# flo-stilz/Audio-Key-Estimation

Measured on AMD Instinct MI355X. Metric: clips/s (15 s @ 22.05 kHz), HIP CQT + PitchClassNet forward, higher is better.
Workload: dtype f32 accumulation everywhere; pitch / semitone / layer-0 convolutions: f16 activations x f16 weights (per-channel power-of-two scaled) on MFMA, one product; last layer's pitch-class convolutions and heads: 3-term split-bf16 on MFMA (hi*hi + lo*hi + hi*lo); CQT filter bank: 3-term split-bf16 on MFMA

## Files before the change

audio-key-estimation_amd/csrc/pcnet.hip:

```cpp
#include <algorithm>
#include <cmath>
#include <cstdlib>
#include <cstring>
#include <map>
#include <string>
#include <vector>

#include "common.h"
#include "pcnet_kernels.h"
#include "pcnet_bwd_kernels.h"

using namespace ake_k;

namespace {

constexpr double kBnEps = 1e-5;
constexpr size_t kLdsBudget = 64 * 1024;
constexpr size_t kBfFragsPerConv = 14 * 2 * 64 + 64;

struct TensorSpec {
    std::string name;
    int64_t shape[4];
    int ndim;
};
// ... 620 lines not shown
        if (j == 0) { a.ph = melh; a.uh = psix_h; a.c0 = 1; a.c1 = c1; a.h1 = 36; }
        else a.xh = planes[j - 1];
        if (!fold) a.oh = planes[j];
        else {
            a.sfrag = n->bf_frags_dev + semi.bf_off; a.sbias = n->blob_dev + semi.b_off;
            a.n_oct = g.n_oct; a.n_units = batch * (36 / a.R);
            a.dst = cat + static_cast<long long>(fold_coff) * 12 * T;
            a.dst_clip_stride = static_cast<long long>(cat_ctot) * 12 * T;
        }
    }
    static ake::DeviceOnce attr_set;
    const int rc = ake::raise_lds_limit(attr_set, 160 * 1024, p2p_stack_kernel);
    if (rc) return rc;
    return ake::launch(name, p2p_stack_kernel, dim3(batch), dim3(1024), g.lds, s, sa);
}

struct P2pX3Plan {
    bool ok = false;
    int R = 0, plane_pos = 0, n_row_tiles = 0, n_tiles = 0, grid = 0;
    size_t lds = 0;
};
P2pX3Plan p2p_f16x3_plan(int c0, int c1, int cout, int batch, int H, int T, bool dst16) {
    P2pX3Plan g;
    if (T < 2 || (T & 1) || c0 < 1 || c0 + c1 > 8 || cout > 8 || batch < 1) return g;
    const int n_cus = device_cus();
    if (n_cus < 8) return g;
    const int Tp = p2p_pitch(T / 2);
    auto plane_of = [&](int R) { return ((R + 6) * Tp + 63) / 64 * 64; };
    auto lds_of = [&](int R) { return (static_cast<size_t>(4) * plane_of(R) + 8 * kP2pMT * kP2pPsStage) * sizeof(uint4); };
    int R = std::max(1, std::min(H, 8 * kP2pMT * 16 / (T / 2)));
    while (R >= 1 && (lds_of(R) > 156 * 1024 || plane_of(R) > 3 * 512)) --R;
    if (R < 1 || H < R + 6) return g;
    if ((R * T) % 4 || (static_cast<long long>(H) * T) % 4 || (static_cast<long long>(cout) * H * T) % 4 || !dst16) return g;
    g.R = R; g.plane_pos = plane_of(R); g.lds = lds_of(R);
    g.n_row_tiles = (H + R - 1) / R;
    g.n_tiles = g.n_row_tiles * batch;
    g.grid = std::min(n_cus / 8 * 8, (g.n_tiles + 7) / 8 * 8);
    g.ok = true;
    return g;
}

struct P2pX3Opts {
    const unsigned int* in_amax = nullptr;
    bool lrelu = false;
};

int run_p2p_f16x3(const ake_pcnet* n, const P2pX3Plan& g, long long frag_off, const Src& src, const float* in_aff, const float* bias, int batch, int H, int T,
                  float* dst, int cout, double* stats, int stats_stride, hipStream_t s, const char* name, const P2pX3Opts& o = {}) {
    AKE_REQUIRE(g.ok && frag_off >= 0 && src.ctot0 == 0, AKE_ERR_STATE, "conv %s: a convolution that does not qualify was sent to the f16 x 3 persistent kernel", name);
    AKE_REQUIRE(g.n_tiles == g.n_row_tiles * batch, AKE_ERR_STATE, "conv %s: the f16 x 3 persistent kernel was planned for another batch than these %d clips", name, batch);
    AKE_REQUIRE(!(reinterpret_cast<uintptr_t>(dst) & 15), AKE_ERR_STATE, "conv %s: the f16 x 3 persistent kernel was planned for 16-byte stores to an unaligned tensor", name);
    P2pTrArgs a;
    std::memset(&a, 0, sizeof(a));
    a.J = T / 2; a.Tp = p2p_pitch(a.J);
    a.R = g.R; a.plane_pos = g.plane_pos;
    a.H = H; a.T = T;
    a.n_row_tiles = g.n_row_tiles; a.n_tiles = g.n_tiles;
    a.p = src.p0; a.c0 = src.c0; a.u = src.p1 ? src.p1 : src.p0; a.c1 = src.p1 ? src.c1 : 0; a.h1 = src.h1 > 0 ? src.h1 : 1;
    a.in_aff = in_aff; a.bfrag = n->bf_frags_dev + frag_off; a.bias = bias;
    a.dst = dst; a.dst_clip_stride = static_cast<long long>(cout) * H * T; a.cout = cout;
    a.stats = stats; a.stats_stride = stats_stride; a.in_amax = o.in_amax; a.lrelu = o.lrelu ? 1 : 0;
    static ake::DeviceOnce attr_set;
    const int rc = ake::raise_lds_limit(attr_set, 160 * 1024, conv_p2p_f16x3_kernel);
    if (rc) return rc;
    return ake::launch(name, conv_p2p_f16x3_kernel, dim3(g.grid), dim3(512), g.lds, s, a);
}

int run_fold_max(const char* label, const float* smap, const float* aff, int C, int S, int batch, int T, float* dst, int dst_ctot, int dst_coff, hipStream_t s) {
    const long long total = static_cast<long long>(batch) * C * 12 * T;
    return launch_flat(label, fold_max_kernel, s, total, smap, aff, C, S, T, dst, static_cast<long long>(dst_ctot) * 12 * T, dst_coff, total);
}

int run_nchw_to_cl16(const float* src, int C, int batch, int T, unsigned short* planes, hipStream_t s) {
    const long long npos = static_cast<long long>(batch) * 12 * T;
    return launch_flat("nchw_to_cl16_kernel", nchw_to_cl16_kernel, s, npos, src, static_cast<long long>(C) * 12 * T, C, T, planes, planes + npos * 16, npos);
}

bool pc2pc_fuses(const ake_pcnet* n, int i, int T) {
    const auto& c = n->cfg;
    if (g_keep_taps || i < 1 || i != c.num_layers - 1 || c.time_pool_size != 2 || c.conv_layers < 1 || c.conv_layers > 4) return false;
    if (!pc2pc_uses_bf16(n, i, T) || T % 4 || 12 * T > 1024 || 3 * ((T + 15) / 16) > 16) return false;
    for (const ConvSite& cs : n->pc2pc[i])
        if (cs.eval.cout != 16 || cs.eval.cin > 16 || cs.eval.kh != 12) return false;
    return (static_cast<size_t>(4) * 12 * (T + 8) * 2 + 2 * 512) * sizeof(uint4) <= 160 * 1024;
}

int run_pc2pc_fused(const ake_pcnet* n, int i, const float* src, int cin, int batch, int T, float* pooled, unsigned short* feat_cl, hipStream_t s) {
    Pc2pcFusedArgs a;
    std::memset(&a, 0, sizeof(a));
    a.src = src; a.src_clip_stride = static_cast<long long>(cin) * 12 * T; a.cin = cin;
    a.n_conv = static_cast<int>(n->pc2pc[i].size());
    for (int j = 0; j < a.n_conv; ++j) { a.bfrag[j] = n->bf_frags_dev + n->pc2pc[i][j].eval.bf_off; a.bias[j] = n->blob_dev + n->pc2pc[i][j].eval.b_off; }
    a.pooled = pooled;
    if (feat_cl) { a.fh = feat_cl; a.fl = feat_cl + static_cast<long long>(batch) * 12 * (T / 2) * 16; }
    a.T = T; a.Tp = T + 8;
    const size_t lds = (static_cast<size_t>(4) * 12 * a.Tp * 2 + 2 * 512) * sizeof(uint4);
    static ake::DeviceOnce attr_set;
    const int rc = ake::raise_lds_limit(attr_set, 160 * 1024, pc2pc_fused_kernel);
    if (rc) return rc;
    return ake::launch("pc2pc_fused_kernel", pc2pc_fused_kernel, dim3(batch), dim3(1024), lds, s, a);
}

bool pc_f16x3_ok(const PackedConv& pt, int T_in, bool same_time) {
    if (pt.bf_off < 0 || pt.cin > 16) return false;
    const int T_out = same_time ? T_in : T_in - pt.kw + 1;
    if (T_out < 1) return false;
    const size_t lds = (static_cast<size_t>(2) * 12 * (T_out + 8) * 2 + 2 * 4 * ((pt.cout + 15) / 16) * 2 * 64) * sizeof(uint4);
    return lds <= 150 * 1024;
}

int run_nchw_to_cl16_f16x2(const float* src, int C, int batch, int T, const float* aff, unsigned short* planes, hipStream_t s, int src_ctot = 0,
                           const unsigned int* amax = nullptr) {
    const long long npos = static_cast<long long>(batch) * 12 * T;
    return launch_flat("nchw_to_cl16_f16x2_kernel", nchw_to_cl16_f16x2_kernel, s, npos, src, static_cast<long long>(src_ctot > 0 ? src_ctot : C) * 12 * T, C, T, aff, planes,
                planes + npos * 16, npos, amax);
}

struct PcBf16Opts {
    const PackedConv* pc2 = nullptr;
    unsigned short* planes_out2 = nullptr;
    bool f16x3 = false;
    double* stats = nullptr;
    int stats_stride = 0;
    const unsigned int* in_amax = nullptr;
};

int run_pc_bf16(const ake_pcnet* n, const PackedConv& pc, const unsigned short* planes_in, int batch, int T_in, bool same_time, bool lrelu,
                float* dst_nchw, unsigned short* planes_out, hipStream_t s, const char* name, const PcBf16Opts& o = {}) {
    PcBfArgs a;
    std::memset(&a, 0, sizeof(a));
    const long long npos_in = static_cast<long long>(batch) * 12 * T_in;
    a.xh = planes_in; a.xl = planes_in + npos_in * 16;
    a.bfrag = n->bf_frags_dev + pc.bf_off; a.bias = n->blob_dev + pc.b_off;
    a.T_in = T_in; a.T_out = same_time ? T_in : T_in - pc.kw + 1; a.pad_l = same_time ? pc.kw / 2 : 0;
    AKE_REQUIRE(a.T_out > 0, AKE_ERR_INVALID, "conv %s: %d frames is too short for the valid head convolutions", name, T_in);
    a.Tp = a.T_out + 8;
    a.cout = pc.cout; a.lrelu = lrelu ? 1 : 0;
    a.KH = pc.kh; a.circular = pc.kh == 12 ? 1 : 0;
    const int H_out = a.circular ? 12 : 12 - pc.kh + 1;
    a.dst = dst_nchw; a.dst_clip_stride = static_cast<long long>(pc.cout) * H_out * a.T_out;
    a.cl_stride = pc.cout;
    if (planes_out) { a.oh = planes_out; a.ol = planes_out + static_cast<long long>(batch) * H_out * a.T_out * pc.cout; }
    if (o.pc2) {
        AKE_REQUIRE(planes_out && o.planes_out2 && o.pc2->cout == pc.cout && o.pc2->kh == pc.kh && o.pc2->kw == pc.kw && o.pc2->cin == pc.cin && o.pc2->bf_off >= 0,
                    AKE_ERR_STATE, "conv %s: the paired convolution differs in shape", name);
        a.bfrag2 = n->bf_frags_dev + o.pc2->bf_off; a.bias2 = n->blob_dev + o.pc2->b_off;
        a.oh2 = o.planes_out2; a.ol2 = o.planes_out2 + static_cast<long long>(batch) * H_out * a.T_out * pc.cout;
    }
    a.stats = o.stats; a.stats_stride = o.stats_stride; a.in_amax = o.in_amax;
    AKE_REQUIRE(!o.f16x3 || (dst_nchw && !planes_out && !o.pc2), AKE_ERR_STATE, "conv %s: the f16 x 3 form writes NCHW f32", name);
    const size_t lds = (static_cast<size_t>(2) * 12 * a.Tp * 2 + 2 * 4 * ((pc.cout + 15) / 16) * 2 * 64) * sizeof(uint4);
    AKE_REQUIRE(lds <= 150 * 1024, AKE_ERR_UNSUPPORTED, "conv %s: %d frames do not fit the bf16 kernel's LDS patch", name, T_in);
    static ake::DeviceOnce attr_set;
    const int rc = ake::raise_lds_limit(attr_set, 150 * 1024, conv_pc_bf16_kernel<1, true>, conv_pc_bf16_kernel<1, false>, conv_pc_bf16_kernel<2, false>,
                                        conv_pc_bf16_kernel<2, true>, conv_pc_bf16_kernel<1, false, true>, conv_pc_bf16_kernel<2, false, true>);
    if (rc) return rc;
    const int tiles = (H_out * a.T_out + 15) / 16;
    const int waves = std::min(8, (tiles + 3) / 4);
    dim3 grid((tiles + waves * 4 - 1) / (waves * 4), o.pc2 ? 2 : 1, batch), block(waves * 64);
    if (o.f16x3 && pc.cout <= 16) return ake::launch(name, conv_pc_bf16_kernel<1, false, true>, grid, block, lds, s, a);
    if (o.f16x3) return ake::launch(name, conv_pc_bf16_kernel<2, false, true>, grid, block, lds, s, a);
    if (pc.cout == 16 && planes_out) return ake::launch(name, conv_pc_bf16_kernel<1, true>, grid, block, lds, s, a);
    if (pc.cout == 16) return ake::launch(name, conv_pc_bf16_kernel<1, false>, grid, block, lds, s, a);
    if (planes_out) return ake::launch(name, conv_pc_bf16_kernel<2, true>, grid, block, lds, s, a);
    return ake::launch(name, conv_pc_bf16_kernel<2, false>, grid, block, lds, s, a);
}

size_t pc_f16x3_full_lds(int T_dz) { return (static_cast<size_t>(2) * 12 * (T_dz + 14) * 2 + 2 * 4 * 2 * 64) * sizeof(uint4); }
bool pc_f16x3_full_ok(int T_dz) { return pc_f16x3_full_lds(T_dz) <= 150 * 1024; }

int run_pc_f16x3_full(const ake_pcnet* n, long long frag_off, int kh, const unsigned short* planes, int batch, int T_dz, float* dst, bool accumulate,
                      hipStream_t s, const char* name, const unsigned int* in_amax = nullptr) {
    PcBfArgs a;
    std::memset(&a, 0, sizeof(a));
    const long long npos_in = static_cast<long long>(batch) * 12 * T_dz;
    a.xh = planes; a.xl = planes + npos_in * 16;
    a.bfrag = n->bf_frags_dev + frag_off; a.bias = nullptr;
    a.T_in = T_dz; a.T_out = T_dz + 6; a.pad_l = 6; a.Tp = a.T_out + 8;
    a.cout = 16; a.lrelu = 0; a.KH = kh; a.circular = kh == 12 ? 1 : 0;
// ... 2143 lines not shown
```

audio-key-estimation_amd/csrc/pcnet_kernels.h:

```cpp
#pragma once

#include <hip/hip_runtime.h>

#include "common.h"

namespace ake_k {

constexpr int TW = 4;
constexpr float kSlope = 0.01f;

struct ConvArgs {
    const float* src0;
    const float* src1;
    long long src0_clip_stride, src1_clip_stride;
    int c0, c1, h1;
    int H;
    int T_in;
    int T_out;
    int H_out;
    int py;
    int pad_l;
    int time_circ;
    const float* w;
    const float* bias;
    int cout;
    float* dst;
    long long dst_clip_stride;
    int dst_coff;
    int lrelu;
    int R;
    int TT;
    int n_row_tiles, n_time_tiles;
    int Tp;
    const float* in_affine;
    double* stats;
    int stats_stride;
    int accumulate;
    const float* residual;
    long long residual_clip_stride;
    int rows_zero;
};

constexpr int kStatSlots = 64;

constexpr double kFxStat = 16777216.0;
constexpr double kFxGrad = 1099511627776.0;
typedef long long gfx_t;
__device__ __forceinline__ void fx_add(long long* cell, double v, double scale) {
    atomicAdd(reinterpret_cast<unsigned long long*>(cell), static_cast<unsigned long long>(__double2ll_rn(v * scale)));
}
__device__ __forceinline__ void fx_add(double* cell, double v, double scale) { fx_add(reinterpret_cast<long long*>(cell), v, scale); }
__device__ __forceinline__ double fx_get(const double* cell, double scale) { return static_cast<double>(*reinterpret_cast<const long long*>(cell)) / scale; }
__device__ __forceinline__ double fx_checked(long long sum, double scale) {
    const long long lim = 1ll << 61;
    return (sum > lim || sum < -lim) ? __longlong_as_double(0x7ff8000000000000ll) : static_cast<double>(sum) / scale;
}

__device__ __forceinline__ void fx_add_int(double* cell, long long v) {
    atomicAdd(reinterpret_cast<unsigned long long*>(cell), static_cast<unsigned long long>(v));
}
struct ShiftStat {
    double s1, s2;
    __device__ __forceinline__ void init() { s1 = 0.0; s2 = 0.0; }
    __device__ __forceinline__ void add(float v) {
        const double d = v;
        s1 += d;
        s2 = fma(d, d, s2);
    }
    __device__ __forceinline__ void fixed(long long& i1, long long& i2) const {
        i1 = __double2ll_rn(s1 * kFxStat);
        i2 = __double2ll_rn(s2 * kFxStat);
    }
};
__device__ __forceinline__ long long shfl_xor_ll(long long v, int o) {
    const int lo = __shfl_xor(static_cast<int>(v & 0xffffffffll), o), hi = __shfl_xor(static_cast<int>(v >> 32), o);
    return (static_cast<long long>(hi) << 32) | static_cast<unsigned int>(lo);
}

__device__ __forceinline__ unsigned int bf16_bits(float v) {
    const unsigned int u = __float_as_uint(v);
    return (u + 0x7FFFu + ((u >> 16) & 1u)) >> 16;
}

__device__ __forceinline__ int wrap(int i, int n) {
    i %= n;
    return i < 0 ? i + n : i;
}

struct SemiArgs {
    const float* src;
    long long src_clip_stride;
    int C, H, T;
    const float* w;
    const float* bias;
    float* dst;
    long long dst_clip_stride;
    int dst_coff;
    int n_strips;
};

template <int CO>
__global__ void semi_fold_kernel(SemiArgs a) {
    const int item = blockIdx.x * blockDim.x + threadIdx.x;
    const int per_clip = 12 * a.n_strips;
    if (item >= per_clip) return;
    const int p = item / a.n_strips;
    const int s = item - p * a.n_strips;
    const int grp = blockIdx.y;
    const int clip = blockIdx.z;
    const int t0 = s * TW;
    int tix[TW + 2];
#pragma unroll
    for (int j = 0; j < TW + 2; ++j) tix[j] = wrap(t0 - 1 + j, a.T);
    const float* src = a.src + clip * a.src_clip_stride;
    const float* __restrict__ wg = a.w + static_cast<long long>(grp) * a.C * (9 * CO);
    float best[CO][TW];
#pragma unroll
    for (int co = 0; co < CO; ++co)
#pragma unroll
        for (int j = 0; j < TW; ++j) best[co][j] = -INFINITY;
    const int n_oct = a.H / 36;
    for (int o = 0; o < n_oct; ++o) {
        const int row0 = 3 * (p + 12 * o);
        float acc[CO][TW];
#pragma unroll
        for (int co = 0; co < CO; ++co)
#pragma unroll
            for (int j = 0; j < TW; ++j) acc[co][j] = 0.f;
        for (int ci = 0; ci < a.C; ++ci) {
#pragma unroll
            for (int dy = 0; dy < 3; ++dy) {
                const float* rowp = src + (static_cast<long long>(ci) * a.H + row0 + dy) * a.T;
                float in[TW + 2];
#pragma unroll
                for (int j = 0; j < TW + 2; ++j) in[j] = rowp[tix[j]];
                const float* __restrict__ wp = wg + (ci * 3 + dy) * (3 * CO);
#pragma unroll
                for (int dx = 0; dx < 3; ++dx)
#pragma unroll
                    for (int co = 0; co < CO; ++co) {
                        const float wv = wp[dx * CO + co];
#pragma unroll
                        for (int j = 0; j < TW; ++j) acc[co][j] = fmaf(in[j + dx], wv, acc[co][j]);
                    }
            }
        }
#pragma unroll
        for (int co = 0; co < CO; ++co) {
            const int c = grp * CO + co;
            const float b = c < a.C ? a.bias[c] : 0.f;
#pragma unroll
            for (int j = 0; j < TW; ++j) {
                float v = acc[co][j] + b;
                v = v > 0.f ? v : v * kSlope;
                best[co][j] = fmaxf(best[co][j], v);
            }
        }
    }
    float* d = a.dst + clip * a.dst_clip_stride;
#pragma unroll
    for (int co = 0; co < CO; ++co) {
        const int c = grp * CO + co;
        if (c >= a.C) break;
        float* drow = d + (static_cast<long long>(a.dst_coff + c) * 12 + p) * a.T;
#pragma unroll
        for (int j = 0; j < TW; ++j)
// ... 1254 lines not shown
            }
        }
        }
        if (dy + 1 < KH) {
            __builtin_amdgcn_s_waitcnt(0x0F70);
            __syncthreads();
        }
    }
#pragma unroll
    for (int mt = 0; mt < MT; ++mt)
#pragma unroll
        for (int nt = 0; nt < NT; ++nt) {
            acc_out[mt][nt] = acc[mt][nt];
            if (F16X3) accl_out[mt][nt] = accl[mt][nt];
        }
}

template <int NT, bool OUT_CL, bool F16X3 = false>
__global__ __launch_bounds__(512) void conv_pc_bf16_kernel(PcBfArgs a) {
    extern __shared__ __attribute__((aligned(16))) uint4 lds4[];
    const int clip = blockIdx.z;
    const int lane = threadIdx.x & 63;
    const int wave = __builtin_amdgcn_readfirstlane(threadIdx.x >> 6);
    const float in_mul = (F16X3 && a.in_amax) ? f16_weight_scale(amax_load(a.in_amax)) : 1.f;
    const int nw = blockDim.x >> 6;
    const int r16 = lane & 15, q = lane >> 4;
    constexpr int MT = 4;
    const int H_out = a.circular ? 12 : 12 - a.KH + 1;
    const int Mtot = H_out * a.T_out;
    const bool second = blockIdx.y == 1;
    const uint4* const bfr = second ? a.bfrag2 : a.bfrag;
    const int tile0 = (blockIdx.x * nw + wave) * MT;
    f32x4c acc[MT][NT], accl[F16X3 ? MT : 1][F16X3 ? NT : 1];
    pc_bf16_multiply<NT, MT, F16X3>(a.xh, a.xl, bfr, lds4, clip, a.T_in, a.T_out, a.pad_l, a.Tp, a.KH, nw, tile0, Mtot, acc, accl);
    if (tile0 * 16 >= Mtot) return;
#pragma unroll
    for (int nt = 0; nt < NT; ++nt) {
        const int co = nt * 16 + r16;
        const float* const bptr = second ? a.bias2 : a.bias;
        const float bias = (co < a.cout && bptr) ? bptr[co] : 0.f;
        float iscale = (F16X3 && co < a.cout) ? reinterpret_cast<const float*>(bfr + a.KH * 4 * NT * 2 * 64)[co] : 1.f;
        if (F16X3 && a.in_amax) iscale /= in_mul;
        ShiftStat sstat;
        sstat.init();
        unsigned short* const oh = second ? a.oh2 : a.oh;
        unsigned short* const ol = second ? a.ol2 : a.ol;
#pragma unroll
        for (int mt = 0; mt < MT; ++mt) {
            const int m0 = (tile0 + mt) * 16 + 4 * q;
            int y = m0 / a.T_out, t = m0 - y * a.T_out;
#pragma unroll
            for (int i = 0; i < 4; ++i) {
                if (m0 + i < Mtot && co < a.cout) {
                    float v = F16X3 ? fmaf(fmaf(accl[F16X3 ? mt : 0][F16X3 ? nt : 0][i], kP2pLoInv, acc[mt][nt][i]), iscale, bias) : acc[mt][nt][i] + bias;
                    if (F16X3) sstat.add(v);
                    if (a.lrelu) v = v > 0.f ? v : v * kSlope;
                    if (OUT_CL) {
                        const long long idx = ((static_cast<long long>(clip) * H_out + y) * a.T_out + t) * a.cl_stride + co;
                        const unsigned int hb = bf16_bits(v);
                        oh[idx] = static_cast<unsigned short>(hb);
                        ol[idx] = static_cast<unsigned short>(bf16_bits(v - __uint_as_float(hb << 16)));
                    } else {
                        float* const d = a.dst + clip * a.dst_clip_stride + (static_cast<long long>(co) * H_out + y) * a.T_out + t;
                        *d = (F16X3 && a.accumulate) ? *d + v : v;
                    }
                }
                if (++t == a.T_out) { t = 0; ++y; }
            }
        }
        if (F16X3 && a.stats) {
            long long st1, st2;
            sstat.fixed(st1, st2);
            st1 += shfl_xor_ll(st1, 16); st2 += shfl_xor_ll(st2, 16);
            st1 += shfl_xor_ll(st1, 32); st2 += shfl_xor_ll(st2, 32);
            if (q == 0 && co < a.cout) {
                double* st = a.stats + static_cast<size_t>((blockIdx.x + 7 * blockIdx.z + wave) & (kStatSlots - 1)) * a.stats_stride;
                fx_add_int(st + 2 * co, st1);
                fx_add_int(st + 2 * co + 1, st2);
            }
        }
    }
}

struct Pc2pcFusedArgs {
    const float* src;
    long long src_clip_stride;
    int cin, n_conv;
    const uint4* bfrag[4];
    const float* bias[4];
    float* pooled;
    unsigned short* fh;
    unsigned short* fl;
    int T, Tp;
};

__global__ __launch_bounds__(1024) void pc2pc_fused_kernel(Pc2pcFusedArgs a) {
    extern __shared__ __attribute__((aligned(16))) uint4 lds4[];
    const int clip = blockIdx.x;
    const int lane = threadIdx.x & 63;
    const int wave = __builtin_amdgcn_readfirstlane(threadIdx.x >> 6);
    const int r16 = lane & 15, q = lane >> 4;
    const int T = a.T, Tp = a.Tp;
    constexpr int MT = 4;
    const int n16 = 12 * Tp * 2;
    uint4* const map0 = lds4;
    uint4* const map1 = lds4 + 2 * n16;
    uint4* const wring = lds4 + 4 * n16;
    constexpr int kRow = 4 * 2 * 64;
    for (int i = threadIdx.x; i < 4 * n16; i += 1024) lds4[i] = make_uint4(0, 0, 0, 0);
    const int wsrc0 = (((threadIdx.x >> 7) * 4) * 2 + ((threadIdx.x >> 6) & 1)) * 64 + (threadIdx.x & 63);
    auto wsrc = [&](int p, int dq) { return wsrc0 + (16 * dq * 2 + p * 2) * 64; };
    if (threadIdx.x < kRow) wring[threadIdx.x] = a.bfrag[0][wsrc(0, 0)];
    __syncthreads();
    {
        const float* src = a.src + clip * a.src_clip_stride;
        for (int i = threadIdx.x; i < 12 * T * 2; i += 1024) {
            const int half = i & 1, pos = i >> 1;
            const int y = pos / T, t = pos - y * T;
            unsigned int hi[4] = {0, 0, 0, 0}, lo[4] = {0, 0, 0, 0};
#pragma unroll
            for (int k = 0; k < 8; ++k) {
                const int c = half * 8 + k;
                const float v = c < a.cin ? src[(static_cast<long long>(c) * 12 + y) * T + t] : 0.f;
                const unsigned int hb = bf16_bits(v);
                hi[k >> 1] |= hb << (16 * (k & 1));
                lo[k >> 1] |= bf16_bits(v - __uint_as_float(hb << 16)) << (16 * (k & 1));
            }
            const int idx = ((y * Tp + t + 3) << 1) + half;
            map0[idx] = make_uint4(hi[0], hi[1], hi[2], hi[3]);
            map0[n16 + idx] = make_uint4(lo[0], lo[1], lo[2], lo[3]);
        }
    }
    __syncthreads();
    const int n_tt = (T + 15) >> 4;
    const bool active = wave < 3 * n_tt;
    const int tt = wave / 3, y0 = 4 * (wave - 3 * tt);
    const int t0 = 16 * tt;
    const int dxq = q >> 1, half = q & 1;
    const int lane_off = ((t0 + r16 + dxq) << 1) + half;
    const int lane_off3 = ((t0 + r16 + 6) << 1) + half;
    auto frag_off = [&](int s, int p) {
        int row = y0 + s + (p == 3 ? dxq : 0);
        row -= row >= 12 ? 12 : 0;
        return ((row * Tp) << 1) + (p == 3 ? lane_off3 : lane_off + 4 * p);
    };
    const int Tf = T / 2;
    float* const pooled_c = a.pooled + static_cast<long long>(clip) * 16 * 12 * Tf;
    unsigned short* const fh_c = a.fh ? a.fh + static_cast<long long>(clip) * 12 * Tf * 16 : nullptr;
    unsigned short* const fl_c = a.fh ? a.fl + static_cast<long long>(clip) * 12 * Tf * 16 : nullptr;
    for (int j = 0; j < a.n_conv; ++j) {
        const uint4* const pH = (j & 1) ? map1 : map0;
        const uint4* const pL = pH + n16;
        unsigned short* const oH = reinterpret_cast<unsigned short*>((j & 1) ? map0 : map1);
        unsigned short* const oL = oH + n16 * 8;
        const bool last = j == a.n_conv - 1;
        const uint4* const bfrag_j = j == 0 ? a.bfrag[0] : (j == 1 ? a.bfrag[1] : (j == 2 ? a.bfrag[2] : a.bfrag[3]));
        const float* const bias_j = j == 0 ? a.bias[0] : (j == 1 ? a.bias[1] : (j == 2 ? a.bias[2] : a.bias[3]));
        const uint4* const bfrag_n = j == 0 ? a.bfrag[1] : (j == 1 ? a.bfrag[2] : a.bfrag[3]);
        {
            f32x4c acc[MT];
#pragma unroll
            for (int mt = 0; mt < MT; ++mt) acc[mt] = f32x4c{0.f, 0.f, 0.f, 0.f};
            bf16x8c fh[4], fl[4];
            int c = 0;
            auto run_p = [&](auto pair_c, const int p) __attribute__((always_inline)) {
                constexpr bool PAIR = decltype(pair_c)::value;
                if (active) {
#pragma unroll
                    for (int s = 0; s < 4; ++s) {
                        const int off = frag_off(s, PAIR ? 3 : p);
                        fh[s] = __builtin_bit_cast(bf16x8c, pH[off]);
                        fl[s] = __builtin_bit_cast(bf16x8c, pL[off]);
                    }
                }
#pragma unroll 1
                for (int dq = 0; dq < 3; ++dq, ++c) {
                    uint4 wpre = make_uint4(0, 0, 0, 0);
                    const bool fetch = threadIdx.x < kRow && (c + 1 < 12 || j + 1 < a.n_conv);
                    if (fetch) wpre = c + 1 < 12 ? bfrag_j[dq < 2 ? wsrc(p, dq + 1) : wsrc(p + 1, 0)] : bfrag_n[wsrc(0, 0)];
                    const uint4* const wr = wring + (c & 1) * kRow + lane;
                    if (active) {
#pragma unroll
                        for (int i = 0; i < 4; i += PAIR ? 2 : 1) {
                            const bf16x8c bh = __builtin_bit_cast(bf16x8c, wr[(i * 2 + 0) * 64]), bl = __builtin_bit_cast(bf16x8c, wr[(i * 2 + 1) * 64]);
#pragma unroll
                            for (int mt = 0; mt < MT; ++mt) acc[mt] = __builtin_amdgcn_mfma_f32_16x16x32_bf16(fh[(mt + i) & 3], bh, acc[mt], 0, 0, 0);
#pragma unroll
                            for (int mt = 0; mt < MT; ++mt) acc[mt] = __builtin_amdgcn_mfma_f32_16x16x32_bf16(fl[(mt + i) & 3], bh, acc[mt], 0, 0, 0);
#pragma unroll
                            for (int mt = 0; mt < MT; ++mt) acc[mt] = __builtin_amdgcn_mfma_f32_16x16x32_bf16(fh[(mt + i) & 3], bl, acc[mt], 0, 0, 0);
#pragma unroll
                            for (int u = 0; u < (PAIR ? 2 : 1); ++u) {
                                const int s_new = 4 * dq + i + 4 + u;
                                if (s_new < 12 + MT - (PAIR ? 2 : 1)) {
                                    const int off = frag_off(s_new, PAIR ? 3 : p);
                                    fh[i + u] = __builtin_bit_cast(bf16x8c, pH[off]);
                                    fl[i + u] = __builtin_bit_cast(bf16x8c, pL[off]);
                                }
                            }
                        }
                    }
                    if (fetch) wring[((c + 1) & 1) * kRow + threadIdx.x] = wpre;
                    if (c + 1 < 12) __syncthreads();
                }
            };
#pragma unroll 1
            for (int p = 0; p < 3; ++p) run_p(std::false_type{}, p);
            run_p(std::true_type{}, 3);
            if (active) {
            const int co = r16;
            const float bias = bias_j[co];
            const int tq0 = t0 + 4 * q;
            if (tq0 < T) {
#pragma unroll
            for (int mt = 0; mt < MT; ++mt) {
                    const int y = y0 + mt;
                    float v[4];
#pragma unroll
                    for (int i = 0; i < 4; ++i) {
                        const float x = acc[mt][i] + bias;
                        v[i] = x > 0.f ? x : x * kSlope;
                    }
                    if (!last) {
#pragma unroll
                        for (int i = 0; i < 4; ++i) {
                            const int e = ((((y * Tp + tq0 + i + 3) << 1) + (co >> 3)) << 3) + (co & 7);
                            const unsigned int hb = bf16_bits(v[i]);
                            oH[e] = static_cast<unsigned short>(hb);
                            oL[e] = static_cast<unsigned short>(bf16_bits(v[i] - __uint_as_float(hb << 16)));
                        }
                    } else {
#pragma unroll
                        for (int i = 0; i < 4; i += 2) {
                            const float pv = fmaxf(v[i], v[i + 1]);
                            const int tq = (tq0 + i) >> 1;
                            pooled_c[(co * 12 + y) * Tf + tq] = pv;
                            if (a.fh) {
                                const int e = (y * Tf + tq) * 16 + co;
                                const unsigned int hb = bf16_bits(pv);
                                fh_c[e] = static_cast<unsigned short>(hb);
                                fl_c[e] = static_cast<unsigned short>(bf16_bits(pv - __uint_as_float(hb << 16)));
                            }
                        }
                    }
            }
            }
            }
        }
        __syncthreads();
    }
}

struct Head1BfArgs {
    const unsigned short* xh[3];
    const unsigned short* xl[3];
    const uint4* bfrag[3];
    const float* bias[3];
    float* dst[3];
    int KH[3], H_out[3], circular[3];
    int T_in, T_out, Tp, JB;
    float* pout[3];
    PoolArgs pool;
    int fin_off;
};

constexpr int kHead1MT = 4;
constexpr int kHead1JB = 5;
__host__ __device__ constexpr int head1_ksteps(int KH) { return KH == 12 ? 12 * 7 : KH * 22; }
constexpr int kHead1PF = 3;

__device__ __forceinline__ void head1_prefetch(const uint4* __restrict__ bg, int nks, int wave, uint4 (&nbh)[kHead1PF], uint4 (&nbl)[kHead1PF]) {
#pragma unroll
    for (int i = 0; i < kHead1PF; ++i) {
        const int kn = wave + 8 * i < nks ? wave + 8 * i : wave;
        nbh[i] = bg[(2 * kn + 0) * 64]; nbl[i] = bg[(2 * kn + 1) * 64];
    }
}

__device__ __forceinline__ void head1_multiply_store(const uint4* __restrict__ bg, int nks, uint4 (&nbh)[kHead1PF], uint4 (&nbl)[kHead1PF], uint4* lds4,
                                                     int Tp, int HO, int circ, int JB, int T_out, int clip, const float* bias_p, float* dst,
                                                     bool keep, int fin_off) {
    constexpr int PF = kHead1PF;
    const int lane = threadIdx.x & 63;
    const int wave = __builtin_amdgcn_readfirstlane(threadIdx.x >> 6);
    const int r16 = lane & 15, q = lane >> 4;
    const uint4* const pH = lds4;
    const uint4* const pL = lds4 + 12 * Tp * 4;
    float* const red = reinterpret_cast<float*>(lds4);
    if (circ) {
        f32x4c acc[kHead1JB];
#pragma unroll
        for (int mt = 0; mt < kHead1JB; ++mt) acc[mt] = f32x4c{0.f, 0.f, 0.f, 0.f};
        for (int ks = wave; ks < nks; ks += 8) {
            const int r = ks / 7, dx = ks - r * 7;
            const bf16x8c bh = __builtin_bit_cast(bf16x8c, nbh[0]);
            const bf16x8c bl = __builtin_bit_cast(bf16x8c, nbl[0]);
#pragma unroll
            for (int i = 0; i + 1 < PF; ++i) { nbh[i] = nbh[i + 1]; nbl[i] = nbl[i + 1]; }
            {
                const int kn = ks + 8 * PF < nks ? ks + 8 * PF : ks;
                nbh[PF - 1] = bg[(2 * kn + 0) * 64]; nbl[PF - 1] = bg[(2 * kn + 1) * 64];
            }
            const int ad0 = ((r * Tp + r16 + dx) << 2) + q;
#pragma unroll
            for (int mt = 0; mt < kHead1JB; ++mt) {
                if (mt < JB) {
                    const bf16x8c ah = __builtin_bit_cast(bf16x8c, pH[ad0 + 64 * mt]);
                    const bf16x8c al = __builtin_bit_cast(bf16x8c, pL[ad0 + 64 * mt]);
                    acc[mt] = __builtin_amdgcn_mfma_f32_16x16x32_bf16(ah, bh, acc[mt], 0, 0, 0);
                    acc[mt] = __builtin_amdgcn_mfma_f32_16x16x32_bf16(al, bh, acc[mt], 0, 0, 0);
                    acc[mt] = __builtin_amdgcn_mfma_f32_16x16x32_bf16(ah, bl, acc[mt], 0, 0, 0);
                }
            }
        }
        __syncthreads();
#pragma unroll
        for (int mt = 0; mt < kHead1JB; ++mt)
            if (mt < JB)
#pragma unroll
                for (int i = 0; i < 4; ++i) red[((wave * JB + mt) * 4 + i) * 64 + lane] = acc[mt][i];
        __syncthreads();
        if (wave < JB) {
            const float bias = bias_p[0];
#pragma unroll
            for (int i = 0; i < 4; ++i) {
                float v = bias;
#pragma unroll
                for (int w = 0; w < 8; ++w) v += red[((w * JB + wave) * 4 + i) * 64 + lane];
                const int t = 16 * wave + 4 * q + i;
                if (r16 < 12 && t < T_out) {
                    dst[(static_cast<long long>(clip) * 12 + r16) * T_out + t] = v;
// ... 1257 lines not shown
```

Before: 504,400.

## Pipeline pc2pc fused weight ring with LDS DMA and register-held weights

Reworks the fused last-layer pitch-class convolution kernel. Weight fragments now stream into a three-slot LDS ring through asynchronous global-to-LDS DMA, issued by half the waves alternately. They are held in registers one chunk ahead, so the old per-thread copy through registers and double-buffered writes go away. MFMA issue is interleaved with fragment reloads using a sched_barrier, the input loads are hoisted, only the halo of the LDS maps is zeroed, and a packed bf16x2 conversion replaces the scalar hi/lo splits. This is intended to hide weight-fetch latency and cut conversion and zero-fill cost, at the price of raw waitcnt/s_barrier synchronisation that is fragile to get right.

```diff
diff --git a/audio-key-estimation_amd/csrc/bf16_split.h b/audio-key-estimation_amd/csrc/bf16_split.h
--- /dev/null
+++ b/audio-key-estimation_amd/csrc/bf16_split.h
@@ -0,0 +1,22 @@
+#pragma once
+
+#include <hip/hip_runtime.h>
+
+namespace ake_k {
+
+__device__ __forceinline__ unsigned int bf16_bits(float v) {
+    const unsigned int u = __float_as_uint(v);
+    return (u + 0x7FFFu + ((u >> 16) & 1u)) >> 16;
+}
+
+typedef float f32x2c __attribute__((ext_vector_type(2)));
+typedef __bf16 bf16x2c __attribute__((ext_vector_type(2)));
+__device__ __forceinline__ void bf16_split2(float a, float b, unsigned int& hi, unsigned int& lo) {
+    const f32x2c v = {a, b};
+    const bf16x2c h = __builtin_convertvector(v, bf16x2c);
+    const f32x2c r = v - __builtin_convertvector(h, f32x2c);
+    hi = __builtin_bit_cast(unsigned int, h);
+    lo = __builtin_bit_cast(unsigned int, __builtin_convertvector(r, bf16x2c));
+}
+
+}
diff --git a/audio-key-estimation_amd/csrc/pcnet.hip b/audio-key-estimation_amd/csrc/pcnet.hip
--- a/audio-key-estimation_amd/csrc/pcnet.hip
+++ b/audio-key-estimation_amd/csrc/pcnet.hip
@@ -726,7 +726,7 @@
     if (!pc2pc_uses_bf16(n, i, T) || T % 4 || 12 * T > 1024 || 3 * ((T + 15) / 16) > 16) return false;
     for (const ConvSite& cs : n->pc2pc[i])
         if (cs.eval.cout != 16 || cs.eval.cin > 16 || cs.eval.kh != 12) return false;
-    return (static_cast<size_t>(4) * 12 * (T + 8) * 2 + 2 * 512) * sizeof(uint4) <= 160 * 1024;
+    return pc2pc_fused_lds_bytes(T) <= 160 * 1024;
 }
 
 int run_pc2pc_fused(const ake_pcnet* n, int i, const float* src, int cin, int batch, int T, float* pooled, unsigned short* feat_cl, hipStream_t s) {
@@ -738,7 +738,7 @@
     a.pooled = pooled;
     if (feat_cl) { a.fh = feat_cl; a.fl = feat_cl + static_cast<long long>(batch) * 12 * (T / 2) * 16; }
     a.T = T; a.Tp = T + 8;
-    const size_t lds = (static_cast<size_t>(4) * 12 * a.Tp * 2 + 2 * 512) * sizeof(uint4);
+    const size_t lds = pc2pc_fused_lds_bytes(T);
     static ake::DeviceOnce attr_set;
     const int rc = ake::raise_lds_limit(attr_set, 160 * 1024, pc2pc_fused_kernel);
     if (rc) return rc;
diff --git a/audio-key-estimation_amd/csrc/pcnet_kernels.h b/audio-key-estimation_amd/csrc/pcnet_kernels.h
--- a/audio-key-estimation_amd/csrc/pcnet_kernels.h
+++ b/audio-key-estimation_amd/csrc/pcnet_kernels.h
@@ -2,6 +2,7 @@
 
 #include <hip/hip_runtime.h>
 
+#include "bf16_split.h"
 #include "common.h"
 
 namespace ake_k {
@@ -77,11 +78,6 @@
     return (static_cast<long long>(hi) << 32) | static_cast<unsigned int>(lo);
 }
 
-__device__ __forceinline__ unsigned int bf16_bits(float v) {
-    const unsigned int u = __float_as_uint(v);
-    return (u + 0x7FFFu + ((u >> 16) & 1u)) >> 16;
-}
-
 __device__ __forceinline__ int wrap(int i, int n) {
     i %= n;
     return i < 0 ? i + n : i;
@@ -1502,6 +1498,13 @@
     }
 }
 
+constexpr int kPc2pcRingSlots = 3;
+constexpr int kPc2pcChunk = 4 * 2 * 64;
+__host__ __device__ constexpr int pc2pc_plane_u4(int T) { return 12 * (T + 8) * 2; }
+__host__ __device__ constexpr size_t pc2pc_fused_lds_bytes(int T) {
+    return (static_cast<size_t>(4) * pc2pc_plane_u4(T) + kPc2pcRingSlots * kPc2pcChunk) * sizeof(uint4);
+}
+
 struct Pc2pcFusedArgs {
     const float* src;
     long long src_clip_stride;
@@ -1522,35 +1525,53 @@
     const int r16 = lane & 15, q = lane >> 4;
     const int T = a.T, Tp = a.Tp;
     constexpr int MT = 4;
-    const int n16 = 12 * Tp * 2;
+    const int n16 = pc2pc_plane_u4(T);
     uint4* const map0 = lds4;
     uint4* const map1 = lds4 + 2 * n16;
     uint4* const wring = lds4 + 4 * n16;
-    constexpr int kRow = 4 * 2 * 64;
-    for (int i = threadIdx.x; i < 4 * n16; i += 1024) lds4[i] = make_uint4(0, 0, 0, 0);
-    const int wsrc0 = (((threadIdx.x >> 7) * 4) * 2 + ((threadIdx.x >> 6) & 1)) * 64 + (threadIdx.x & 63);
-    auto wsrc = [&](int p, int dq) { return wsrc0 + (16 * dq * 2 + p * 2) * 64; };
-    if (threadIdx.x < kRow) wring[threadIdx.x] = a.bfrag[0][wsrc(0, 0)];
-    __syncthreads();
+    const unsigned int ring_lds = static_cast<unsigned int>(reinterpret_cast<unsigned long long>(wring));
+    auto request = [&](const uint4* bfr, int p, int dq) {
+        if ((wave >> 3) == ((p + dq) & 1)) {
+            const int piece = wave & 7;
+            ake::lds_dma_16(bfr + (((4 * dq + (piece >> 1)) * 4 + p) * 2 + (piece & 1)) * 64 + lane,
+                            ring_lds + static_cast<unsigned int>((dq * kPc2pcChunk + piece * 64) * sizeof(uint4)));
+        }
+    };
+    request(a.bfrag[0], 0, 0);
+    request(a.bfrag[0], 0, 1);
     {
         const float* src = a.src + clip * a.src_clip_stride;
-        for (int i = threadIdx.x; i < 12 * T * 2; i += 1024) {
+        const int nitem = 12 * T * 2;
+        float xin[2][8];
+#pragma unroll
+        for (int r = 0; r < 2; ++r) {
+            const int i = min(static_cast<int>(threadIdx.x) + 1024 * r, nitem - 1);
+            const int half = i & 1, pos = i >> 1;
+#pragma unroll
+            for (int k = 0; k < 8; ++k) xin[r][k] = src[min(half * 8 + k, a.cin - 1) * (12 * T) + pos];
+        }
+        if (threadIdx.x < 4 * 12 * 16) {
+            const int plane = threadIdx.x / 192, rem = threadIdx.x - plane * 192;
+            const int row = rem >> 4, k = rem & 15;
+            lds4[plane * n16 + row * Tp * 2 + (k < 6 ? k : (T + 3) * 2 + k - 6)] = make_uint4(0, 0, 0, 0);
+        }
+#pragma unroll
+        for (int r = 0; r < 2; ++r) {
+            const int i = threadIdx.x + 1024 * r;
             const int half = i & 1, pos = i >> 1;
             const int y = pos / T, t = pos - y * T;
-            unsigned int hi[4] = {0, 0, 0, 0}, lo[4] = {0, 0, 0, 0};
-#pragma unroll
-            for (int k = 0; k < 8; ++k) {
-                const int c = half * 8 + k;
-                const float v = c < a.cin ? src[(static_cast<long long>(c) * 12 + y) * T + t] : 0.f;
-                const unsigned int hb = bf16_bits(v);
-                hi[k >> 1] |= hb << (16 * (k & 1));
-                lo[k >> 1] |= bf16_bits(v - __uint_as_float(hb << 16)) << (16 * (k & 1));
-            }
-            const int idx = ((y * Tp + t + 3) << 1) + half;
-            map0[idx] = make_uint4(hi[0], hi[1], hi[2], hi[3]);
-            map0[n16 + idx] = make_uint4(lo[0], lo[1], lo[2], lo[3]);
-        }
-    }
+            unsigned int hi[4], lo[4];
+#pragma unroll
+            for (int k = 0; k < 8; k += 2)
+                bf16_split2(half * 8 + k < a.cin ? xin[r][k] : 0.f, half * 8 + k + 1 < a.cin ? xin[r][k + 1] : 0.f, hi[k >> 1], lo[k >> 1]);
+            if (i < nitem) {
+                const int idx = ((y * Tp + t + 3) << 1) + half;
+                map0[idx] = make_uint4(hi[0], hi[1], hi[2], hi[3]);
+                map0[n16 + idx] = make_uint4(lo[0], lo[1], lo[2], lo[3]);
+            }
+        }
+    }
+    __builtin_amdgcn_s_waitcnt(0x0F70);
     __syncthreads();
     const int n_tt = (T + 15) >> 4;
     const bool active = wave < 3 * n_tt;
@@ -1568,6 +1589,14 @@
     float* const pooled_c = a.pooled + static_cast<long long>(clip) * 16 * 12 * Tf;
     unsigned short* const fh_c = a.fh ? a.fh + static_cast<long long>(clip) * 12 * Tf * 16 : nullptr;
     unsigned short* const fl_c = a.fh ? a.fl + static_cast<long long>(clip) * 12 * Tf * 16 : nullptr;
+    uint4 bw[4][2];
+    if (active) {
+#pragma unroll
+        for (int i = 0; i < 4; ++i) {
+            bw[i][0] = wring[(i * 2 + 0) * 64 + lane];
+            bw[i][1] = wring[(i * 2 + 1) * 64 + lane];
+        }
+    }
     for (int j = 0; j < a.n_conv; ++j) {
         const uint4* const pH = (j & 1) ? map1 : map0;
         const uint4* const pL = pH + n16;
@@ -1582,7 +1611,6 @@
 #pragma unroll
             for (int mt = 0; mt < MT; ++mt) acc[mt] = f32x4c{0.f, 0.f, 0.f, 0.f};
             bf16x8c fh[4], fl[4];
-            int c = 0;
             auto run_p = [&](auto pair_c, const int p) __attribute__((always_inline)) {
                 constexpr bool PAIR = decltype(pair_c)::value;
                 if (active) {
@@ -1594,34 +1622,46 @@
                     }
                 }
 #pragma unroll 1
-                for (int dq = 0; dq < 3; ++dq, ++c) {
-                    uint4 wpre = make_uint4(0, 0, 0, 0);
-                    const bool fetch = threadIdx.x < kRow && (c + 1 < 12 || j + 1 < a.n_conv);
-                    if (fetch) wpre = c + 1 < 12 ? bfrag_j[dq < 2 ? wsrc(p, dq + 1) : wsrc(p + 1, 0)] : bfrag_n[wsrc(0, 0)];
-                    const uint4* const wr = wring + (c & 1) * kRow + lane;
+                for (int dq = 0; dq < 3; ++dq) {
+                    {
+                        const int dq2 = dq == 0 ? 2 : dq - 1, p2 = p + (dq > 0);
+                        if (!PAIR || dq == 0) request(bfrag_j, p2, dq2);
+                        else if (j + 1 < a.n_conv) request(bfrag_n, 0, dq2);
+                    }
+                    const uint4* const wn = wring + (dq == 2 ? 0 : dq + 1) * kPc2pcChunk + lane;
                     if (active) {
 #pragma unroll
                         for (int i = 0; i < 4; i += PAIR ? 2 : 1) {
-                            const bf16x8c bh = __builtin_bit_cast(bf16x8c, wr[(i * 2 + 0) * 64]), bl = __builtin_bit_cast(bf16x8c, wr[(i * 2 + 1) * 64]);
+                            const bf16x8c bh = __builtin_bit_cast(bf16x8c, bw[i][0]), bl = __builtin_bit_cast(bf16x8c, bw[i][1]);
+                            int off_new[PAIR ? 2 : 1];
+#pragma unroll
+                            for (int u = 0; u < (PAIR ? 2 : 1); ++u) off_new[u] = frag_off(min(4 * dq + i + 4 + u, 12 + MT - (PAIR ? 2 : 1) - 1), PAIR ? 3 : p);
 #pragma unroll
                             for (int mt = 0; mt < MT; ++mt) acc[mt] = __builtin_amdgcn_mfma_f32_16x16x32_bf16(fh[(mt + i) & 3], bh, acc[mt], 0, 0, 0);
 #pragma unroll
                             for (int mt = 0; mt < MT; ++mt) acc[mt] = __builtin_amdgcn_mfma_f32_16x16x32_bf16(fl[(mt + i) & 3], bh, acc[mt], 0, 0, 0);
-#pragma unroll
-                            for (int mt = 0; mt < MT; ++mt) acc[mt] = __builtin_amdgcn_mfma_f32_16x16x32_bf16(fh[(mt + i) & 3], bl, acc[mt], 0, 0, 0);
-#pragma unroll
-                            for (int u = 0; u < (PAIR ? 2 : 1); ++u) {
-                                const int s_new = 4 * dq + i + 4 + u;
-                                if (s_new < 12 + MT - (PAIR ? 2 : 1)) {
-                                    const int off = frag_off(s_new, PAIR ? 3 : p);
-                                    fh[i + u] = __builtin_bit_cast(bf16x8c, pH[off]);
-                                    fl[i + u] = __builtin_bit_cast(bf16x8c, pL[off]);
-                                }
+                            constexpr int kFree = PAIR ? 2 : 1;
+#pragma unroll
+                            for (int mt = 0; mt < kFree; ++mt) acc[mt] = __builtin_amdgcn_mfma_f32_16x16x32_bf16(fh[(mt + i) & 3], bl, acc[mt], 0, 0, 0);
+#pragma unroll
+                            for (int u = 0; u < kFree; ++u) {
+                                fh[i + u] = __builtin_bit_cast(bf16x8c, pH[off_new[u]]);
+                                fl[i + u] = __builtin_bit_cast(bf16x8c, pL[off_new[u]]);
+                            }
+                            __builtin_amdgcn_sched_barrier(0);
+#pragma unroll
+                            for (int mt = kFree; mt < MT; ++mt) acc[mt] = __builtin_amdgcn_mfma_f32_16x16x32_bf16(fh[(mt + i) & 3], bl, acc[mt], 0, 0, 0);
+#pragma unroll
+                            for (int u = 0; u < kFree; ++u) {
+                                bw[i + u][0] = wn[((i + u) * 2 + 0) * 64];
+                                bw[i + u][1] = wn[((i + u) * 2 + 1) * 64];
                             }
                         }
                     }
-                    if (fetch) wring[((c + 1) & 1) * kRow + threadIdx.x] = wpre;
-                    if (c + 1 < 12) __syncthreads();
+                    if (!PAIR || dq < 2) {
+                        __builtin_amdgcn_s_waitcnt(0x0F70);
+                        asm volatile("s_barrier" ::: "memory");
+                    }
                 }
             };
 #pragma unroll 1
@@ -1632,9 +1672,11 @@
             const float bias = bias_j[co];
             const int tq0 = t0 + 4 * q;
             if (tq0 < T) {
-#pragma unroll
-            for (int mt = 0; mt < MT; ++mt) {
-                    const int y = y0 + mt;
+                int e = ((y0 * Tp + tq0 + 3) << 4) + co;
+                int g = (co * 12 + y0) * Tf + (tq0 >> 1);
+                int ec = (y0 * Tf + (tq0 >> 1)) * 16 + co;
+#pragma unroll
+                for (int mt = 0; mt < MT; ++mt, e += Tp * 16, g += Tf, ec += Tf * 16) {
                     float v[4];
 #pragma unroll
                     for (int i = 0; i < 4; ++i) {
@@ -1643,30 +1685,32 @@
                     }
                     if (!last) {
 #pragma unroll
-                        for (int i = 0; i < 4; ++i) {
-                            const int e = ((((y * Tp + tq0 + i + 3) << 1) + (co >> 3)) << 3) + (co & 7);
-                            const unsigned int hb = bf16_bits(v[i]);
-                            oH[e] = static_cast<unsigned short>(hb);
-                            oL[e] = static_cast<unsigned short>(bf16_bits(v[i] - __uint_as_float(hb << 16)));
+                        for (int i = 0; i < 4; i += 2) {
+                            unsigned int hi, lo;
+                            bf16_split2(v[i], v[i + 1], hi, lo);
+                            oH[e + 16 * i] = static_cast<unsigned short>(hi);
+                            oH[e + 16 * i + 16] = static_cast<unsigned short>(hi >> 16);
+                            oL[e + 16 * i] = static_cast<unsigned short>(lo);
+                            oL[e + 16 * i + 16] = static_cast<unsigned short>(lo >> 16);
                         }
                     } else {
-#pragma unroll
-                        for (int i = 0; i < 4; i += 2) {
-                            const float pv = fmaxf(v[i], v[i + 1]);
-                            const int tq = (tq0 + i) >> 1;
-                            pooled_c[(co * 12 + y) * Tf + tq] = pv;
-                            if (a.fh) {
-                                const int e = (y * Tf + tq) * 16 + co;
-                                const unsigned int hb = bf16_bits(pv);
-                                fh_c[e] = static_cast<unsigned short>(hb);
-                                fl_c[e] = static_cast<unsigned short>(bf16_bits(pv - __uint_as_float(hb << 16)));
-                            }
+                        const float pv0 = fmaxf(v[0], v[1]), pv1 = fmaxf(v[2], v[3]);
+                        pooled_c[g] = pv0;
+                        pooled_c[g + 1] = pv1;
+                        if (a.fh) {
+                            unsigned int hi, lo;
+                            bf16_split2(pv0, pv1, hi, lo);
+                            fh_c[ec] = static_cast<unsigned short>(hi);
+                            fh_c[ec + 16] = static_cast<unsigned short>(hi >> 16);
+                            fl_c[ec] = static_cast<unsigned short>(lo);
+                            fl_c[ec + 16] = static_cast<unsigned short>(lo >> 16);
                         }
                     }
-            }
-            }
-            }
-        }
+                }
+            }
+            }
+        }
+        if (!last) __builtin_amdgcn_s_waitcnt(0x0F70);
         __syncthreads();
     }
 }
```

Result: faster. 512,800 (median of 6 runs) (+1.7%).
